# Excalibur-SLE/wave-fenics

Measured on AMD Instinct MI355X. Metric: dofs/sec stiffness-operator apply, P4 hex box mesh, higher is better.
Workload: dtype f64; 1 GPU; P4 hex box 54^3 cells, 10218313 dofs, stiffness + lumped-mass-inverse apply; degree=4, cells_per_gpu=157464, global_dofs=10218313, parallelism=single, kernel=box

## Files before the change

wave_fenics_amd/build.py:

```python
from __future__ import annotations

import os
import subprocess
import sys

HERE = os.path.dirname(os.path.abspath(__file__))
ROOT = os.path.dirname(HERE)
CSRC = os.path.join(HERE, "csrc")
LIB = os.path.join(HERE, "libwavehip.so")
SOURCES = [
    "tables.cpp", "mesh_io.cpp", "generic_plan.cpp", "box_run_plan.cpp", "function_space.cpp", "box_space.cpp", "markers.cpp",
    "hex_geometry.hip", "stiffness_batch.hip", "mass_batch.hip", "stiffness_march.hip", "stiffness_march_owner.hip", "stiffness_march_idx.hip", "stiffness_march_ks.hip",
    "mass_march.hip", "ordered.hip", "stiffness_dense.hip", "mass_dense_simplex.hip", "tsmm.hip", "vector_kernels.hip", "comm.hip", "cg.hip", "api.hip",
    "hex_cell_geometry.cpp", "op_setup.hip", "op_create.hip", "op_create_box.hip", "op_apply.hip",
]
HEADERS = [os.path.join(CSRC, "common.h"), os.path.join(CSRC, "device_array.h"), os.path.join(CSRC, "op.h"),
           os.path.join(CSRC, "stiffness_core.h"), os.path.join(CSRC, "cell_batch.h"), os.path.join(CSRC, "stiffness_elementwise.h"),
           os.path.join(CSRC, "march_column.h"), os.path.join(CSRC, "box_run_plan.h"), os.path.join(CSRC, "dense_simplex.h"),
           os.path.join(ROOT, "include", "wavehip.h")]


def hipcc() -> str:
    for cand in (os.environ.get("HIPCC"), "/opt/rocm/bin/hipcc", "hipcc"):
        if cand and (os.path.isabs(cand) and os.path.exists(cand) or not os.path.isabs(cand)):
            return cand
    raise RuntimeError("hipcc not found")


def needs_build() -> bool:
    if not os.path.exists(LIB):
        return True
    t = os.path.getmtime(LIB)
    deps = [os.path.join(CSRC, s) for s in SOURCES] + HEADERS
    return any(os.path.getmtime(d) > t for d in deps)


def _compile(src: str, force: bool, verbose: bool) -> str:
    obj = os.path.join(CSRC, os.path.splitext(src)[0] + ".o")
    path = os.path.join(CSRC, src)
    deps = [path] + HEADERS
    if not force and os.path.exists(obj) and all(os.path.getmtime(d) <= os.path.getmtime(obj) for d in deps):
        return obj
    cmd = [hipcc(), "--offload-arch=gfx950", "-O3", "-std=c++17", "-fPIC", "-munsafe-fp-atomics",
           "-I",
           os.path.join(ROOT, "include"), "-I", CSRC, "-c", path, "-o", obj]
    if verbose:
        cmd.insert(1, "-Rpass-analysis=kernel-resource-usage")
    subprocess.check_call(cmd)
    return obj


def build(force: bool = False, verbose: bool = False) -> str:
    if not force and not needs_build():
        return LIB
    from concurrent.futures import ThreadPoolExecutor
    with ThreadPoolExecutor(max_workers=1 if verbose else min(8, len(SOURCES))) as ex:
        objs = list(ex.map(lambda s: _compile(s, force, verbose), SOURCES))
    subprocess.check_call([hipcc(), "--offload-arch=gfx950", "-shared", "-fPIC", "-o", LIB] + objs + ["-ldl"])
    return LIB


if __name__ == "__main__":
    print(build(force="--force" in sys.argv, verbose="--verbose" in sys.argv))
```

wave_fenics_amd/csrc/stiffness_march_owner.hip:

```cpp
#include <cstdlib>

#include "march_column.h"
#include "stiffness_core.h"

namespace wf {

#ifndef WF_OWNER_WAVES
#define WF_OWNER_WAVES 3
#endif
#ifndef WF_OWNER_WAVES_HI
#define WF_OWNER_WAVES_HI 2
#endif

template <int P>
constexpr int owner_waves() { return P >= 5 ? WF_OWNER_WAVES_HI : WF_OWNER_WAVES; }

#ifndef WF_OWNER_LANE_EXCHANGE
#define WF_OWNER_LANE_EXCHANGE 1
#endif

template <int P>
constexpr bool owner_lane_exchange() { return WF_OWNER_LANE_EXCHANGE != 0 && P == 4; }

template <int P, int BX, int BY>
constexpr int owner_lane_line(int t)
{
  const int c = 4 * (t / 64) + (t % 64) / 16, j = (t % 16) / 4, i = t % 4;
  return P * (c % BX) + i + P * BX * (P * (c / BX) + j);
}

template <int P, int BX, int BY>
constexpr bool owner_lane_map_is_bijection()
{
  if (P != 4 || BX * BY != 16) return false;
  bool seen[256] = {};
  for (int t = 0; t < 256; ++t) {
    const int l = owner_lane_line<P, BX, BY>(t);
    if (l < 0 || l >= P * BX * P * BY || seen[l]) return false;
    seen[l] = true;
  }
  return true;
}

template <int CTRL>
__device__ __forceinline__ double dpp_move(double v)
{
  const int lo = __builtin_amdgcn_mov_dpp(__double2loint(v), CTRL, 0xf, 0xf, false);
  const int hi = __builtin_amdgcn_mov_dpp(__double2hiint(v), CTRL, 0xf, 0xf, false);
  return __hiloint2double(hi, lo);
}
__device__ __forceinline__ double add_rounded(double a, double b)
{
#pragma clang fp contract(off)
  return a + b;
}
constexpr int dpp_quad(int a) { return a | a << 2 | a << 4 | a << 6; }
constexpr int dpp_row_ror(int n) { return 0x120 + n; }

template <int P, int BX, int BY>
__global__ __launch_bounds__(256, (owner_waves<P>())) void k_stiffness_owner(
    int nx, int ny, int nz, int lz, int lz0, int gbx, int gby, const double* __restrict__ Gc, const double* __restrict__ dD, DMat am,
    double coeff, const double* __restrict__ x, double* __restrict__ y, const int32_t* __restrict__ items,
    int ablate_arg)
{
  [[maybe_unused]] const int ablate = WF_ABLATE_FLAGS(ablate_arg);
  constexpr int n = P + 1;
  constexpr int LX = P * BX, LY = P * BY, NL = LX * LY;
  constexpr int RX = LX + P + 1, RY = LY + P + 1, RP = RX * RY;
  constexpr int NPF = (P * RP + 255) / 256;
  constexpr int NCP = (RP + 255) / 256;
  constexpr int GCX = BX + 1, GC = GCX * (BY + 1), NG = 3 * GC;
  constexpr int NGL = (NG + 255) / 256;
  static_assert(NL <= 256, "column does not fit a 256-thread workgroup");
  constexpr bool lx = owner_lane_exchange<P>();
  static_assert(!lx || owner_lane_map_is_bijection<P, BX, BY>(), "lane-exchange map is not onto the owned lines");

  __shared__ __attribute__((aligned(16))) double Ux[(P + 1) * RP + 256];
  __shared__ __attribute__((aligned(16))) double Gs[NGL * 256];
#ifdef WF_OWNER_A_CONST
  constexpr bool a_lds = false, a_const = P >= 5;
#else
  constexpr bool a_lds = P >= 5, a_const = false;
#endif
  __shared__ __attribute__((aligned(16))) double As[a_lds ? P * n : 1];
  auto arow = [&](int k, int a) {
    if (a_const) return dD[2 * n * n + n + k * n + a];
    if (a_lds && k < P) return As[k * n + a];
    return am.v[k * n + a];
  };

  const int t = threadIdx.x;
  const int NX = P * nx + 1, NY = P * ny + 1;
  const size_t plane = (size_t)NX * NY;
  const int nbxo = (NX + LX - 1) / LX, nbyo = (NY + LY - 1) / LY, ncols = nbxo * nbyo;
  const bool table = lz < 0;
  const int nwg = (int)gridDim.x, xq = nwg / 8, xr = nwg % 8, xcd = (int)blockIdx.x % 8;
  const int b = (xcd < xr ? xcd * (xq + 1) : xr * (xq + 1) + (xcd - xr) * xq) + (int)blockIdx.x / 8;
  const int e = table ? 3 * (int)blockIdx.x : b;
  const int w0 = items ? items[e] : b;
  const int w1 = table ? items[e + 1] : 0, w2 = table ? items[e + 2] : 0;
  const BoxSegment zs = box_segment(w0 / ncols, nz, lz, lz0);
  const int col = table ? w0 : w0 % ncols, z0 = table ? w1 : zs.z0, z1 = table ? w2 : zs.z1;
  const int Bx = col % nbxo, By = col / nbxo;
  const int I0 = LX * Bx, J0 = LY * By, cx0 = BX * Bx, cy0 = BY * By;

  const int tt = lx ? owner_lane_line<P, BX, BY>(t) : t < NL ? t : NL - 1;
  const int ti = tt % LX, tj = tt / LX, i = ti % P, j = tj % P;
  const int I = I0 + ti, J = J0 + tj;
  const bool own = t < NL && I < NX && J < NY;
  const int32_t yoff = own ? (int32_t)((size_t)I + (size_t)NX * J) : (int32_t)((size_t)I0 + (size_t)NX * J0);
  const int rown = (tj + P) * RX, cown = ti + P;
  const int cR = P + ti - i, rA = P + tj - j;

  double ai[n], aj[n], wk[n];
#pragma unroll
  for (int a = 0; a < n; ++a) {
    wk[a] = dD[2 * n * n + a];
    ai[a] = dD[2 * n * n + n + i * n + a];
    aj[a] = dD[2 * n * n + n + j * n + a];
  }
  const double cwj = coeff * wk[j], cwi = coeff * wk[i], cwij = coeff * wk[i] * wk[j];
  if constexpr (a_lds)
    if (t < P * n) As[t] = dD[2 * n * n + n + t];
  [[maybe_unused]] double ajr[n];
  if constexpr (lx) {
    const int js[P] = {j, __builtin_amdgcn_mov_dpp(j, dpp_row_ror(4), 0xf, 0xf, false),
                       __builtin_amdgcn_mov_dpp(j, dpp_row_ror(8), 0xf, 0xf, false),
                       __builtin_amdgcn_mov_dpp(j, dpp_row_ror(12), 0xf, 0xf, false)};
#pragma unroll
    for (int m = 0; m < P; ++m) ajr[m] = dD[2 * n * n + n + j * n + js[m]];
    ajr[P] = aj[P];
  }

  int32_t poff[NPF];
#pragma unroll
  for (int m = 0; m < NPF; ++m) {
    const int pos = t + 256 * m;
    const int pl = pos / RP, r = pos % RP, II = I0 - P + r % RX, JJ = J0 - P + r / RX;
    poff[m] = -1;
    if (pos < P * RP && II >= 0 && II < NX && JJ >= 0 && JJ < NY)
      poff[m] = (int32_t)((size_t)II + (size_t)NX * JJ + plane * pl);
  }
  const int32_t pclamp = (int32_t)((size_t)I0 + (size_t)NX * J0);

  const int nbx = (nx + gbx - 1) / gbx, nby = (ny + gby - 1) / gby;
  const size_t gstride = (size_t)nbx * nby * (gbx * gby) * 6;
  size_t gbase[NGL];
  bool gval[NGL];
#pragma unroll
  for (int q = 0; q < NGL; ++q) {
    const int e = t + 256 * q, comp = e / GC, c = e % GC;
    const int cx = cx0 - 1 + c % GCX, cy = cy0 - 1 + c / GCX;
    gval[q] = e < NG && cx >= 0 && cx < nx && cy >= 0 && cy < ny;
    const int cxc = gval[q] ? cx : 0, cyc = gval[q] ? cy : 0;
    gbase[q] = (((size_t)(cxc / gbx) + (size_t)nbx * (cyc / gby)) * (gbx * gby) + cxc % gbx + gbx * (cyc % gby)) * 6 +
               (comp == 0 ? 0 : comp == 1 ? 3 : 5);
  }
  auto load_g = [&](double (&g)[NGL], int kz) {
#pragma unroll
    for (int q = 0; q < NGL; ++q) g[q] = Gc[gbase[q] + gstride * kz];
  };
  auto store_g = [&](const double (&g)[NGL]) {
#pragma unroll
    for (int q = 0; q < NGL; ++q) Gs[t + 256 * q] = gval[q] ? g[q] : 0.0;
  };
  const bool mi = i == 0, mj = j == 0;
  const int lR = (ti - i) / P + 1, lA = (tj - j) / P + 1;
  auto scales = [&](double (&s)[5]) {
    const double* g0 = Gs;
    const double* g1 = Gs + GC;
    const double* g2 = Gs + 2 * GC;
    const int AR = lA * GCX + lR, AL = AR - 1, BR = AR - GCX, BL = BR - 1;
    const double x_ar = g0[AR], x_br = g0[BR], x_al = g0[AL], x_bl = g0[BL];
    const double y_ar = g1[AR], y_al = g1[AL], y_br = g1[BR], y_bl = g1[BL];
    const double z_ar = g2[AR], z_al = g2[AL], z_br = g2[BR], z_bl = g2[BL];
    s[0] = cwj * (mj ? x_ar + x_br : x_ar);
    s[1] = mi ? cwj * (mj ? x_al + x_bl : x_al) : 0.0;
    s[2] = cwi * (mi ? y_ar + y_al : y_ar);
    s[3] = mj ? cwi * (mi ? y_br + y_bl : y_br) : 0.0;
    const double za = mi ? z_ar + z_al : z_ar, zb = mi ? z_br + z_bl : z_br;
    s[4] = cwij * (mj ? za + zb : za);
  };

  double xz[2 * P + 1];
  double sc[5], sf[4], spz;
  double yA[P], yB[P];
  {
    double gp[NGL], gcur[NGL];
    load_g(gp, z0 > 0 ? z0 - 1 : z0);
    load_g(gcur, z0);
#pragma unroll
    for (int m = 0; m < P; ++m) {
      const long K = (long)P * z0 - P + m;
      const double v = x[plane * (size_t)(K >= 0 ? K : 0) + yoff];
      xz[m] = K >= 0 ? v : 0.0;
    }
#pragma unroll
    for (int k = 0; k < P; ++k) yA[k] = (ablate & 1) ? 0.0 : y[plane * (size_t)(P * z0 + k) + yoff];
    const double* xb = x + plane * (size_t)(P * z0) + plane;
    double xp0[NCP], xp[NPF];
#pragma unroll
    for (int m = 0; m < NCP; ++m) xp0[m] = (xb - plane)[t + 256 * m < RP && poff[m] >= 0 ? poff[m] : pclamp];
#pragma unroll
    for (int m = 0; m < NPF; ++m) xp[m] = xb[poff[m] >= 0 ? poff[m] : pclamp];
#pragma unroll
    for (int m = 0; m < NCP; ++m) {
      const int pos = t + 256 * m;
      Ux[tile_or_dump<RP>(m, pos, 0, (P + 1) * RP, t)] = (pos < RP && poff[m] >= 0) ? xp0[m] : 0.0;
    }
#pragma unroll
    for (int m = 0; m < NPF; ++m) {
      const int pos = t + 256 * m;
      Ux[tile_or_dump<P * RP>(m, pos, RP, (P + 1) * RP, t)] = poff[m] >= 0 ? xp[m] : 0.0;
    }
    store_g(gp);
    __syncthreads();
    double sp[5];
    scales(sp);
    if (z0 == 0)
#pragma unroll
      for (int q = 0; q < 5; ++q) sp[q] = 0.0;
    __syncthreads();
    store_g(gcur);
    __syncthreads();
    scales(sc);
#pragma unroll
    for (int q = 0; q < 4; ++q) sf[q] = lx ? add_rounded(sc[q], sp[q]) : sc[q] + sp[q];
    spz = sp[4];
#pragma unroll
    for (int m = 0; m <= P; ++m) xz[P + m] = Ux[m * RP + rown + cown];
  }
  [[maybe_unused]] double zpc = 0.0;
  if constexpr (lx) {
#pragma unroll
    for (int a = 0; a < n; ++a) zpc += arow(P, a) * xz[a];
  }

  if (ablate & 16) {
    double u = zpc + spz;
#pragma unroll
    for (int m = 0; m <= 2 * P; ++m) u += xz[m];
#pragma unroll
    for (int q = 0; q < 5; ++q) u += sc[q];
#pragma unroll
    for (int q = 0; q < 4; ++q) u += sf[q];
#pragma unroll
    for (int k = 0; k < P; ++k) u += yA[k];
    if (u == 1.2345e300) y[yoff] = u;
    return;
  }

  auto xy_terms = [&](int k, double s0, double s1, double s2, double s3) {
    const double* L = Ux + k * RP;
    double xr = 0.0, xl = 0.0, ya = 0.0, yb = 0.0;
    if constexpr (lx) {
      const double xo = xz[P + k];
      const double xc = L[rown + cR + P], yc = L[(rA + P) * RX + cown];
      double vl[P], vb[P];
#pragma unroll
      for (int a = 0; a < P; ++a) vl[a] = vb[a] = 0.0;
      if (mi)
#pragma unroll
        for (int a = 0; a < P; ++a) vl[a] = L[rown + cR - P + a];
      if (mj)
#pragma unroll
        for (int a = 0; a < P; ++a) vb[a] = L[(rA - P + a) * RX + cown];
#pragma unroll
      for (int a = 0; a < P; ++a) {
        xl += arow(P, a) * vl[a];
        yb += arow(P, a) * vb[a];
      }
      xl += arow(P, P) * (mi ? xo : 0.0);
      yb += arow(P, P) * (mj ? xo : 0.0);
      asm volatile("" : "+v"(xl), "+v"(yb));
      xr += ai[0] * dpp_move<dpp_quad(0)>(xo);
      xr += ai[1] * dpp_move<dpp_quad(1)>(xo);
      xr += ai[2] * dpp_move<dpp_quad(2)>(xo);
      xr += ai[3] * dpp_move<dpp_quad(3)>(xo);
      xr += ai[P] * xc;
      ya += ajr[0] * xo;
      ya += ajr[1] * dpp_move<dpp_row_ror(4)>(xo);
      ya += ajr[2] * dpp_move<dpp_row_ror(8)>(xo);
      ya += ajr[3] * dpp_move<dpp_row_ror(12)>(xo);
      ya += ajr[P] * yc;
    } else {
#pragma unroll
      for (int a = 0; a < n; ++a) {
        xr += ai[a] * L[rown + cR + a];
        xl += arow(P, a) * L[rown + cR - P + a];
        ya += aj[a] * L[(rA + a) * RX + cown];
        yb += arow(P, a) * L[(rA - P + a) * RX + cown];
      }
    }
    return xr * s0 + xl * s1 + ya * s2 + yb * s3;
  };
  auto store_y = [&](size_t K, double v) {
    double* dst = y + plane * K + yoff;
    if (ablate & 1) {
      if (v == 1.2345e300) *dst = v;
    } else if (own) {
      *dst = v;
    }
  };

  auto layer = [&](auto hn_tag, double (&ycur)[P], double (&ynext)[P], int kz) {
    constexpr bool has_next = decltype(hn_tag)::value;
    [[maybe_unused]] double xn[NPF], gn[NGL];
    if constexpr (has_next) {
      const double* xb = x + plane * (size_t)(P * (kz + 1) + 1);
#pragma unroll
      for (int m = 0; m < NPF; ++m) xn[m] = xb[poff[m] >= 0 ? poff[m] : pclamp];
      load_g(gn, kz + 1);
#pragma unroll
      for (int k = 0; k < P; ++k) ynext[k] = (ablate & 1) ? 0.0 : y[plane * (size_t)(P * (kz + 1) + k) + yoff];
    }

#pragma unroll
    for (int k = 0; k < P; ++k) {
      double zc = 0.0;
#pragma unroll
      for (int a = 0; a < n; ++a) zc += arow(k, a) * xz[P + a];
      double v;
      if (k == 0) {
        double zp = 0.0;
        if constexpr (lx) {
          zp = zpc;
        } else {
#pragma unroll
          for (int a = 0; a < n; ++a) zp += arow(P, a) * xz[a];
        }
        v = wk[0] * xy_terms(0, sf[0], sf[1], sf[2], sf[3]) + zc * sc[4] + zp * spz;
      } else {
        v = wk[k] * xy_terms(k, sc[0], sc[1], sc[2], sc[3]) + zc * sc[4];
      }
      store_y((size_t)(P * kz + k), ycur[k] + v);
    }

    if constexpr (has_next) {
      if constexpr (lx) {
        zpc = 0.0;
#pragma unroll
        for (int a = 0; a < n; ++a) zpc += arow(P, a) * xz[P + a];
      }
      double xcp[NCP];
#pragma unroll
      for (int m = 0; m < NCP; ++m) {
        const int pos = t + 256 * m;
        xcp[m] = pos < RP ? Ux[P * RP + pos] : 0.0;
      }
      __syncthreads();
#pragma unroll
      for (int m = 0; m < NCP; ++m) {
        const int pos = t + 256 * m;
        Ux[tile_or_dump<RP>(m, pos, 0, (P + 1) * RP, t)] = xcp[m];
      }
#pragma unroll
      for (int m = 0; m < NPF; ++m) {
        const int pos = t + 256 * m;
        Ux[tile_or_dump<P * RP>(m, pos, RP, (P + 1) * RP, t)] = poff[m] >= 0 ? xn[m] : 0.0;
      }
      store_g(gn);
      __syncthreads();
#pragma unroll
      for (int m = 0; m <= P; ++m) xz[m] = xz[m + P];
#pragma unroll
      for (int m = 1; m <= P; ++m) xz[P + m] = Ux[m * RP + rown + cown];
      double sn[5];
      scales(sn);
#pragma unroll
      for (int q = 0; q < 4; ++q) sf[q] = lx ? add_rounded(sn[q], sc[q]) : sn[q] + sc[q];
      spz = sc[4];
#pragma unroll
      for (int q = 0; q < 5; ++q) sc[q] = sn[q];
    }
  };

  for (int kz = z0; kz < z1; kz += 2) {
    if (kz + 1 < z1) {
      layer(On{}, yA, yB, kz);
      if (kz + 2 < z1)
        layer(On{}, yB, yA, kz + 1);
      else
        layer(Off{}, yB, yA, kz + 1);
    } else {
      layer(Off{}, yA, yB, kz);
    }
  }

  if (z1 == nz) {
    double zp = 0.0;
#pragma unroll
    for (int a = 0; a < n; ++a) zp += arow(P, a) * xz[P + a];
    const double v = wk[0] * xy_terms(P, sc[0], sc[1], sc[2], sc[3]) + zp * sc[4];
    const size_t K = (size_t)P * nz;
    const double y0 = (ablate & 1) ? 0.0 : y[plane * K + yoff];
    store_y(K, y0 + v);
  }
}

template <int P, int BX, int BY>
static int launch_owner_t(int nx, int ny, int nz, int lz, int lz0, int gbx, int gby, const double* d_Gcell, const double* d_D,
                          const DMat& am, double coeff, const double* d_x, double* d_y, const int32_t* d_items, int nitems,
                          hipStream_t s)
{
  const int nwg = d_items ? nitems : box_owner_columns(P, nx, ny, BX, BY).count() * box_segments(nz, lz, lz0);
  if (nwg == 0) return WF_OK;
  hipLaunchKernelGGL((k_stiffness_owner<P, BX, BY>), dim3((unsigned)nwg), dim3(256), 0, s, nx, ny, nz, lz, lz0, gbx, gby, d_Gcell,
                     d_D, am, coeff, d_x, d_y, d_items, ablate_flags());
  return launch_status("stiffness_march (owner)");
}

#define WF_OWNER_SHAPES(X)                                                                                \
  X(1, 0, 16, 16) X(1, 1, 32, 8) X(1, 2, 8, 32)                                          \
  X(2, 0, 8, 8) X(2, 1, 16, 4) X(2, 2, 4, 16)                                            \
  X(3, 0, 5, 5) X(3, 1, 7, 3) X(3, 2, 3, 7)                                  \
  X(4, 0, 4, 4) X(4, 1, 8, 2) X(4, 2, 2, 8)      \
  X(5, 0, 3, 3) X(5, 1, 5, 2) X(5, 2, 2, 5)           \
  X(6, 0, 3, 2) X(6, 1, 7, 1) X(6, 2, 2, 3)           \
  X(7, 0, 2, 2) X(7, 1, 5, 1) X(7, 2, 1, 5)

bool march_owner_variant(int P, int variant, int* bx, int* by)
{
#define X(PP, V, BXX, BYY) \
  if (P == PP && variant == V) return *bx = BXX, *by = BYY, true;
  WF_OWNER_SHAPES(X)
#undef X
  return false;
}

int launch_stiffness_march_owner(int P, int variant, int nx, int ny, int nz, int lz, int lz0, int gbx, int gby,
                                 const double* d_Gcell,
                                 const double* d_D, const DMat& am, double coeff, const double* d_x, double* d_y,
                                 const int32_t* d_items, int nitems, hipStream_t s)
{
  if ((size_t)nx * ny * nz == 0) return WF_OK;
#define X(PP, V, BXX, BYY) \
  if (P == PP && variant == V) return launch_owner_t<PP, BXX, BYY>(nx, ny, nz, lz, lz0, gbx, gby, d_Gcell, d_D, am, coeff, d_x, d_y, d_items, nitems, s);
  WF_OWNER_SHAPES(X)
#undef X
  set_error("stiffness_march (owner): unsupported degree/variant");
  return WF_ERR_UNSUPPORTED;
}

int march_owner_resident(int P, int variant)
{
#define X(PP, V, BXX, BYY) \
  if (P == PP && variant == V) return resident_workgroups(k_stiffness_owner<PP, BXX, BYY>);
  WF_OWNER_SHAPES(X)
#undef X
  return 0;
}

}
```

Measured before the change: 119.1 billion dofs/s.

## Stream x planes into double-buffered LDS via global_load_lds in owner march

For P=4, the owner-march stiffness kernel now loads each z-slab of x straight into LDS with 16-byte global_load_lds pieces, one per thread, and handles boundary-straddling pieces with scalar loads. The LDS tile and geometry buffers are double-buffered, so the next layer's loads land in the other buffer. This drops the register staging and the extra barrier around the tile copy. In exchange it doubles LDS use, which may lower occupancy, and adds padding and bookkeeping to select the active buffer.

```diff
diff --git a/wave_fenics_amd/build.py b/wave_fenics_amd/build.py
--- a/wave_fenics_amd/build.py
+++ b/wave_fenics_amd/build.py
@@ -16,7 +16,7 @@
 ]
 HEADERS = [os.path.join(CSRC, "common.h"), os.path.join(CSRC, "device_array.h"), os.path.join(CSRC, "op.h"),
            os.path.join(CSRC, "stiffness_core.h"), os.path.join(CSRC, "cell_batch.h"), os.path.join(CSRC, "stiffness_elementwise.h"),
-           os.path.join(CSRC, "march_column.h"), os.path.join(CSRC, "box_run_plan.h"), os.path.join(CSRC, "dense_simplex.h"),
+           os.path.join(CSRC, "march_column.h"), os.path.join(CSRC, "box_run_plan.h"), os.path.join(CSRC, "dense_simplex.h"), os.path.join(CSRC, "owner_pieces.h"),
            os.path.join(ROOT, "include", "wavehip.h")]
 
 
diff --git a/wave_fenics_amd/csrc/owner_pieces.h b/wave_fenics_amd/csrc/owner_pieces.h
--- /dev/null
+++ b/wave_fenics_amd/csrc/owner_pieces.h
@@ -0,0 +1,49 @@
+#pragma once
+
+#if defined(__HIPCC__) || defined(__CUDACC__)
+#define WF_PIECE_FN __host__ __device__ inline
+#else
+#define WF_PIECE_FN inline
+#endif
+
+namespace wf {
+
+enum OwnerPieceKind { PIECE_NONE = 0, PIECE_OUTSIDE = 1, PIECE_INSIDE = 2, PIECE_STRADDLING = 3 };
+
+struct OwnerRect {
+  int RX, RY, NPC;
+};
+constexpr OwnerRect owner_rect(int P, int BX, int BY)
+{
+  const int rx = P * BX + P + 1, RX = rx + (rx & 1), RY = P * BY + P + 1;
+  return {RX, RY, RX * RY / 2};
+}
+
+struct OwnerPiece {
+  int kind;
+  int half;
+  int off;
+};
+
+WF_PIECE_FN OwnerPiece owner_piece(int P, int BX, int BY, int NX, int NY, int I0, int J0, int q)
+{
+  const OwnerRect R = owner_rect(P, BX, BY);
+  OwnerPiece p = {PIECE_NONE, 0, 0};
+  if (q < 0 || q >= R.NPC) return p;
+  const int hr = R.RX / 2, II = I0 - P + 2 * (q % hr), JJ = J0 - P + q / hr;
+  const bool row = JJ >= 0 && JJ < NY;
+  const bool in0 = row && II >= 0 && II < NX, in1 = row && II + 1 >= 0 && II + 1 < NX;
+  if (in0 && in1) {
+    p.kind = PIECE_INSIDE;
+    p.off = II + NX * JJ;
+  } else if (in0 || in1) {
+    p.kind = PIECE_STRADDLING;
+    p.half = in1 ? 1 : 0;
+    p.off = II + p.half + NX * JJ;
+  } else {
+    p.kind = PIECE_OUTSIDE;
+  }
+  return p;
+}
+
+}
diff --git a/wave_fenics_amd/csrc/stiffness_march_owner.hip b/wave_fenics_amd/csrc/stiffness_march_owner.hip
--- a/wave_fenics_amd/csrc/stiffness_march_owner.hip
+++ b/wave_fenics_amd/csrc/stiffness_march_owner.hip
@@ -1,6 +1,7 @@
 #include <cstdlib>
 
 #include "march_column.h"
+#include "owner_pieces.h"
 #include "stiffness_core.h"
 
 namespace wf {
@@ -22,6 +23,19 @@
 template <int P>
 constexpr bool owner_lane_exchange() { return WF_OWNER_LANE_EXCHANGE != 0 && P == 4; }
 
+#ifndef WF_OWNER_DMA
+#define WF_OWNER_DMA 1
+#endif
+
+template <int P, int BX, int BY>
+constexpr bool owner_dma() { return WF_OWNER_DMA != 0 && P == 4 && owner_rect(P, BX, BY).NPC <= 256; }
+
+__device__ __forceinline__ void load_to_lds16(const double* src, double* dst)
+{
+  __builtin_amdgcn_global_load_lds((const __attribute__((address_space(1))) void*)src,
+                                   (__attribute__((address_space(3))) void*)dst, 16, 0, 0);
+}
+
 template <int P, int BX, int BY>
 constexpr int owner_lane_line(int t)
 {
@@ -66,17 +80,21 @@
   [[maybe_unused]] const int ablate = WF_ABLATE_FLAGS(ablate_arg);
   constexpr int n = P + 1;
   constexpr int LX = P * BX, LY = P * BY, NL = LX * LY;
-  constexpr int RX = LX + P + 1, RY = LY + P + 1, RP = RX * RY;
+  constexpr bool dma = owner_dma<P, BX, BY>();
+  constexpr int NB = dma ? 2 : 1;
+  constexpr int RX = dma ? owner_rect(P, BX, BY).RX : LX + P + 1, RY = LY + P + 1, RP = RX * RY;
+  constexpr int NPC = RP / 2, UB = (P + 1) * RP;
   constexpr int NPF = (P * RP + 255) / 256;
   constexpr int NCP = (RP + 255) / 256;
   constexpr int GCX = BX + 1, GC = GCX * (BY + 1), NG = 3 * GC;
   constexpr int NGL = (NG + 255) / 256;
   static_assert(NL <= 256, "column does not fit a 256-thread workgroup");
+  static_assert(!dma || (RP % 2 == 0 && NPC <= 256), "a plane is not one 16-byte piece per thread");
   constexpr bool lx = owner_lane_exchange<P>();
   static_assert(!lx || owner_lane_map_is_bijection<P, BX, BY>(), "lane-exchange map is not onto the owned lines");
 
-  __shared__ __attribute__((aligned(16))) double Ux[(P + 1) * RP + 256];
-  __shared__ __attribute__((aligned(16))) double Gs[NGL * 256];
+  __shared__ __attribute__((aligned(16))) double Ux[dma ? NB * UB : UB + 256];
+  __shared__ __attribute__((aligned(16))) double Gs[NB * NGL * 256];
 #ifdef WF_OWNER_A_CONST
   constexpr bool a_lds = false, a_const = P >= 5;
 #else
@@ -142,6 +160,9 @@
       poff[m] = (int32_t)((size_t)II + (size_t)NX * JJ + plane * pl);
   }
   const int32_t pclamp = (int32_t)((size_t)I0 + (size_t)NX * J0);
+  [[maybe_unused]] const OwnerPiece pc = dma ? owner_piece(P, BX, BY, NX, NY, I0, J0, t) : OwnerPiece{PIECE_NONE, 0, 0};
+  [[maybe_unused]] const bool pc_in = pc.kind == PIECE_INSIDE, pc_edge = pc.kind == PIECE_STRADDLING;
+  [[maybe_unused]] double* const wave_img = dma ? Ux + 128 * __builtin_amdgcn_readfirstlane(t >> 6) : Ux;
 
   const int nbx = (nx + gbx - 1) / gbx, nby = (ny + gby - 1) / gby;
   const size_t gstride = (size_t)nbx * nby * (gbx * gby) * 6;
@@ -160,16 +181,21 @@
 #pragma unroll
     for (int q = 0; q < NGL; ++q) g[q] = Gc[gbase[q] + gstride * kz];
   };
-  auto store_g = [&](const double (&g)[NGL]) {
-#pragma unroll
-    for (int q = 0; q < NGL; ++q) Gs[t + 256 * q] = gval[q] ? g[q] : 0.0;
+  auto store_g = [&](const double (&g)[NGL], int gb = 0) {
+#pragma unroll
+    for (int q = 0; q < NGL; ++q)
+      if constexpr (dma)
+        Gs[gb * (NGL * 256) + t + 256 * q] = gval[q] ? g[q] : 0.0;
+      else
+        Gs[t + 256 * q] = gval[q] ? g[q] : 0.0;
   };
   const bool mi = i == 0, mj = j == 0;
   const int lR = (ti - i) / P + 1, lA = (tj - j) / P + 1;
-  auto scales = [&](double (&s)[5]) {
+  auto scales = [&](double (&s)[5], int gb = 0) {
     const double* g0 = Gs;
     const double* g1 = Gs + GC;
     const double* g2 = Gs + 2 * GC;
+    if constexpr (dma) g0 += gb * (NGL * 256), g1 += gb * (NGL * 256), g2 += gb * (NGL * 256);
     const int AR = lA * GCX + lR, AL = AR - 1, BR = AR - GCX, BL = BR - 1;
     const double x_ar = g0[AR], x_br = g0[BR], x_al = g0[AL], x_bl = g0[BL];
     const double y_ar = g1[AR], y_al = g1[AL], y_br = g1[BR], y_bl = g1[BL];
@@ -197,21 +223,38 @@
     }
 #pragma unroll
     for (int k = 0; k < P; ++k) yA[k] = (ablate & 1) ? 0.0 : y[plane * (size_t)(P * z0 + k) + yoff];
-    const double* xb = x + plane * (size_t)(P * z0) + plane;
-    double xp0[NCP], xp[NPF];
-#pragma unroll
-    for (int m = 0; m < NCP; ++m) xp0[m] = (xb - plane)[t + 256 * m < RP && poff[m] >= 0 ? poff[m] : pclamp];
-#pragma unroll
-    for (int m = 0; m < NPF; ++m) xp[m] = xb[poff[m] >= 0 ? poff[m] : pclamp];
-#pragma unroll
-    for (int m = 0; m < NCP; ++m) {
-      const int pos = t + 256 * m;
-      Ux[tile_or_dump<RP>(m, pos, 0, (P + 1) * RP, t)] = (pos < RP && poff[m] >= 0) ? xp0[m] : 0.0;
-    }
-#pragma unroll
-    for (int m = 0; m < NPF; ++m) {
-      const int pos = t + 256 * m;
-      Ux[tile_or_dump<P * RP>(m, pos, RP, (P + 1) * RP, t)] = poff[m] >= 0 ? xp[m] : 0.0;
+    if constexpr (dma) {
+      if (pc.kind == PIECE_OUTSIDE || pc_edge)
+#pragma unroll
+        for (int m = 0; m < NB * (P + 1); ++m) Ux[m * RP + 2 * t] = Ux[m * RP + 2 * t + 1] = 0.0;
+      const double* xb = x + plane * (size_t)(P * z0) + pc.off;
+      if (pc_in)
+#pragma unroll
+        for (int m = 0; m <= P; ++m) load_to_lds16(xb + plane * m, wave_img + m * RP);
+      if (pc_edge) {
+        double xe[P + 1];
+#pragma unroll
+        for (int m = 0; m <= P; ++m) xe[m] = xb[plane * m];
+#pragma unroll
+        for (int m = 0; m <= P; ++m) Ux[m * RP + 2 * t + pc.half] = xe[m];
+      }
+    } else {
+      const double* xb = x + plane * (size_t)(P * z0) + plane;
+      double xp0[NCP], xp[NPF];
+#pragma unroll
+      for (int m = 0; m < NCP; ++m) xp0[m] = (xb - plane)[t + 256 * m < RP && poff[m] >= 0 ? poff[m] : pclamp];
+#pragma unroll
+      for (int m = 0; m < NPF; ++m) xp[m] = xb[poff[m] >= 0 ? poff[m] : pclamp];
+#pragma unroll
+      for (int m = 0; m < NCP; ++m) {
+        const int pos = t + 256 * m;
+        Ux[tile_or_dump<RP>(m, pos, 0, (P + 1) * RP, t)] = (pos < RP && poff[m] >= 0) ? xp0[m] : 0.0;
+      }
+#pragma unroll
+      for (int m = 0; m < NPF; ++m) {
+        const int pos = t + 256 * m;
+        Ux[tile_or_dump<P * RP>(m, pos, RP, (P + 1) * RP, t)] = poff[m] >= 0 ? xp[m] : 0.0;
+      }
     }
     store_g(gp);
     __syncthreads();
@@ -250,8 +293,9 @@
     return;
   }
 
-  auto xy_terms = [&](int k, double s0, double s1, double s2, double s3) {
+  auto xy_terms = [&](int k, double s0, double s1, double s2, double s3, int cb = 0) {
     const double* L = Ux + k * RP;
+    if constexpr (dma) L += cb * UB;
     double xr = 0.0, xl = 0.0, ya = 0.0, yb = 0.0;
     if constexpr (lx) {
       const double xo = xz[P + k];
@@ -303,13 +347,23 @@
     }
   };
 
-  auto layer = [&](auto hn_tag, double (&ycur)[P], double (&ynext)[P], int kz) {
+  auto layer = [&](auto hn_tag, double (&ycur)[P], double (&ynext)[P], int kz, int cb = 0) {
     constexpr bool has_next = decltype(hn_tag)::value;
-    [[maybe_unused]] double xn[NPF], gn[NGL];
+    [[maybe_unused]] const int nb = 1 - cb;
+    [[maybe_unused]] double xn[NPF], gn[NGL], xe[P];
     if constexpr (has_next) {
       const double* xb = x + plane * (size_t)(P * (kz + 1) + 1);
-#pragma unroll
-      for (int m = 0; m < NPF; ++m) xn[m] = xb[poff[m] >= 0 ? poff[m] : pclamp];
+      if constexpr (dma) {
+        if (pc_in)
+#pragma unroll
+          for (int m = 0; m < P; ++m) load_to_lds16(xb + plane * m + pc.off, wave_img + nb * UB + (m + 1) * RP);
+        if (pc_edge)
+#pragma unroll
+          for (int m = 0; m < P; ++m) xe[m] = xb[plane * m + pc.off];
+      } else {
+#pragma unroll
+        for (int m = 0; m < NPF; ++m) xn[m] = xb[poff[m] >= 0 ? poff[m] : pclamp];
+      }
       load_g(gn, kz + 1);
 #pragma unroll
       for (int k = 0; k < P; ++k) ynext[k] = (ablate & 1) ? 0.0 : y[plane * (size_t)(P * (kz + 1) + k) + yoff];
@@ -329,9 +383,9 @@
 #pragma unroll
           for (int a = 0; a < n; ++a) zp += arow(P, a) * xz[a];
         }
-        v = wk[0] * xy_terms(0, sf[0], sf[1], sf[2], sf[3]) + zc * sc[4] + zp * spz;
+        v = wk[0] * xy_terms(0, sf[0], sf[1], sf[2], sf[3], cb) + zc * sc[4] + zp * spz;
       } else {
-        v = wk[k] * xy_terms(k, sc[0], sc[1], sc[2], sc[3]) + zc * sc[4];
+        v = wk[k] * xy_terms(k, sc[0], sc[1], sc[2], sc[3], cb) + zc * sc[4];
       }
       store_y((size_t)(P * kz + k), ycur[k] + v);
     }
@@ -342,31 +396,46 @@
 #pragma unroll
         for (int a = 0; a < n; ++a) zpc += arow(P, a) * xz[P + a];
       }
-      double xcp[NCP];
-#pragma unroll
-      for (int m = 0; m < NCP; ++m) {
-        const int pos = t + 256 * m;
-        xcp[m] = pos < RP ? Ux[P * RP + pos] : 0.0;
-      }
+      if constexpr (dma) {
+        if (t < NPC) {
+          const double c0 = Ux[cb * UB + P * RP + 2 * t], c1 = Ux[cb * UB + P * RP + 2 * t + 1];
+          Ux[nb * UB + 2 * t] = c0;
+          Ux[nb * UB + 2 * t + 1] = c1;
+        }
+        if (pc_edge)
+#pragma unroll
+          for (int m = 0; m < P; ++m) Ux[nb * UB + (m + 1) * RP + 2 * t + pc.half] = xe[m];
+      } else {
+        double xcp[NCP];
+#pragma unroll
+        for (int m = 0; m < NCP; ++m) {
+          const int pos = t + 256 * m;
+          xcp[m] = pos < RP ? Ux[P * RP + pos] : 0.0;
+        }
+        __syncthreads();
+#pragma unroll
+        for (int m = 0; m < NCP; ++m) {
+          const int pos = t + 256 * m;
+          Ux[tile_or_dump<RP>(m, pos, 0, (P + 1) * RP, t)] = xcp[m];
+        }
+#pragma unroll
+        for (int m = 0; m < NPF; ++m) {
+          const int pos = t + 256 * m;
+          Ux[tile_or_dump<P * RP>(m, pos, RP, (P + 1) * RP, t)] = poff[m] >= 0 ? xn[m] : 0.0;
+        }
+      }
+      store_g(gn, nb);
       __syncthreads();
 #pragma unroll
-      for (int m = 0; m < NCP; ++m) {
-        const int pos = t + 256 * m;
-        Ux[tile_or_dump<RP>(m, pos, 0, (P + 1) * RP, t)] = xcp[m];
-      }
-#pragma unroll
-      for (int m = 0; m < NPF; ++m) {
-        const int pos = t + 256 * m;
-        Ux[tile_or_dump<P * RP>(m, pos, RP, (P + 1) * RP, t)] = poff[m] >= 0 ? xn[m] : 0.0;
-      }
-      store_g(gn);
-      __syncthreads();
-#pragma unroll
       for (int m = 0; m <= P; ++m) xz[m] = xz[m + P];
 #pragma unroll
-      for (int m = 1; m <= P; ++m) xz[P + m] = Ux[m * RP + rown + cown];
+      for (int m = 1; m <= P; ++m)
+        if constexpr (dma)
+          xz[P + m] = Ux[nb * UB + m * RP + rown + cown];
+        else
+          xz[P + m] = Ux[m * RP + rown + cown];
       double sn[5];
-      scales(sn);
+      scales(sn, nb);
 #pragma unroll
       for (int q = 0; q < 4; ++q) sf[q] = lx ? add_rounded(sn[q], sc[q]) : sn[q] + sc[q];
       spz = sc[4];
@@ -377,13 +446,13 @@
 
   for (int kz = z0; kz < z1; kz += 2) {
     if (kz + 1 < z1) {
-      layer(On{}, yA, yB, kz);
+      layer(On{}, yA, yB, kz, 0);
       if (kz + 2 < z1)
-        layer(On{}, yB, yA, kz + 1);
+        layer(On{}, yB, yA, kz + 1, dma ? 1 : 0);
       else
-        layer(Off{}, yB, yA, kz + 1);
+        layer(Off{}, yB, yA, kz + 1, dma ? 1 : 0);
     } else {
-      layer(Off{}, yA, yB, kz);
+      layer(Off{}, yA, yB, kz, 0);
     }
   }
 
@@ -391,7 +460,12 @@
     double zp = 0.0;
 #pragma unroll
     for (int a = 0; a < n; ++a) zp += arow(P, a) * xz[P + a];
-    const double v = wk[0] * xy_terms(P, sc[0], sc[1], sc[2], sc[3]) + zp * sc[4];
+    double xy;
+    if constexpr (dma)
+      xy = ((z1 - z0) & 1) ? xy_terms(P, sc[0], sc[1], sc[2], sc[3], 0) : xy_terms(P, sc[0], sc[1], sc[2], sc[3], 1);
+    else
+      xy = xy_terms(P, sc[0], sc[1], sc[2], sc[3]);
+    const double v = wk[0] * xy + zp * sc[4];
     const size_t K = (size_t)P * nz;
     const double y0 = (ablate & 1) ? 0.0 : y[plane * K + yoff];
     store_y(K, y0 + v);
```

After: 121.7 billion dofs/s (median of 6 runs). 1.02x the previous value.
